# AnnSeidel/genometools

Measured on AMD Instinct MI355X. Metric: Gbp/s ESA build (suf+lcp+bwt), 3 Gbp DNA, 1/2/4/8 MI355X; bit-exact vs CPU, higher is better.
Workload: dtype u64; 1 GPU; human-like DNA (2% N, 24 seqs, repeats) n=3000000000 seed=43 -suf -lcp -bwt (BASELINE.json configs[2]); parallelism=1 device, pair_suffixes=341032298, tied_suffixes=390540711, refine_rounds=9, maxbranchdepth=8256

## Files before the change

### genometools_amd/csrc/esa_engine.hip

```cpp
#include <stdarg.h>
#include <stdlib.h>
#include <chrono>
#include <type_traits>
#include <utility>
#include <vector>
#include "../../include/gtamd_esa.h"
#include "esa_prims.h"
#include "esa_devutil.h"
#include "esa_own.h"

static thread_local char g_err[1024] = "";
void gtamd_set_error(const char *fmt, ...) {
  va_list ap;
  va_start(ap, fmt);
  vsnprintf(g_err, sizeof g_err, fmt, ap);
  va_end(ap);
}
extern "C" const char *gtamd_esa_last_error(void) { return g_err; }

extern "C" int gtamd_device_count(void) {
  GTAMD_ABI_BEGIN
  int n = 0;
  if (hipGetDeviceCount(&n) != hipSuccess) return 0;
  return n;
  GTAMD_ABI_END(0)
}

extern "C" int gtamd_abi_selftest(uint64_t host_bytes) {
  GTAMD_ABI_BEGIN
  std::vector<u8> probe((size_t) host_bytes);
  if (!probe.empty()) probe[probe.size() - 1] = 1;
  return probe.empty() ? 0 : (int) probe[probe.size() - 1] - 1;
  GTAMD_ABI_END(-1)
}

// ... 2449 lines not shown
  if (const char *e = getenv("GTAMD_APPLY_EARLY")) sw.apply_early = atoi(e);
  if (sw.apply_early < 0 || sw.apply_early > 2) sw.apply_early = 0;
  if (const char *e = getenv("GTAMD_APPLY_WGS")) {
    const long v = atol(e);
    if (v >= 64 && v <= (1 << 22)) sw.apply_wgs = (u64) v;
    sw.apply_wgs_given = true;
  }
  if (const char *e = getenv("GTAMD_RANK_WINDOW_BITS")) {
    const int v = atoi(e);
    if (v >= 2 && v <= RW_BITS) sw.rank_window_bits = v;
  }
  sw.rank_all_windows = flag("GTAMD_RANK_ALL_WINDOWS", '1');
  sw.win_filter_global = flag("GTAMD_WIN_FILTER_LDS", '0');
  if (const char *e = getenv("GTAMD_PAIR_CHUNK")) {
    const int v = atoi(e);
    if (v >= 4 && v <= 1024) sw.pair_chunk = v;
  }
  if (const char *e = getenv("GTAMD_ROUND_STRIDE")) {
    const int v = atoi(e);
    if (v >= RT_STRIDE_MIN && v <= RT_TILE) sw.round_stride = (u32) v;
  }
  sw.debug = getenv("GTAMD_DEBUG") != nullptr;
  return sw;
}

struct gtamd_esa_ctx {
  int device = 0;
  u32 sigma = 0;
  int bits = 0;
  u64 max_n = 0, n = 0, N = 0;
  int readmode = 0;
  Stream st, st2;
  Event ev_sorted, ev_emitted, ev_applied;
  DevBuf tb_own, sp_own;
  Text text = {};
  bool have_text = false;
  DevBuf k0, k1, v0, v1;
  DevBuf isa_tmp;
  DevBuf rws;
  DevBuf msd;
  DevBuf suf, lcp, bwt;
  DevBuf tiebits, tiebits2;
  DevBuf arena;
  DevBuf arena_p;
  DevBuf xrecv;
  DevBuf winbuf;
  DevBuf lcpfull_buf;
  DevBuf partws;
  DevBuf posw;
  Dev<u64> llv;
  u64 llv_pairs = 0;
  Dev<u32> bck;
  u64 bck_codes = 0, bck_special = 0, bck_dist = 0;
  Dev<Stats> d_stats;
  Pinned<Stats> h_stats;
  Pinned<u32> h_counts;
  Pinned<u32> h_hist;
  u32 user_prefixlength = 0;
  u32 part = 0, numparts = 1;
  gtamd_allgather_fn comm_allgather = nullptr;
  gtamd_alltoallv_fn comm_alltoallv = nullptr;
  void (*comm_abort)(void *) = nullptr;
  void *comm_abort_user = nullptr;
  void *comm_user = nullptr;
  u64 NL = 0, index_offset = 0;
  Dev<u32> d_parthist;
// ... 37 lines not shown
                    "context holds %llu bytes already, %llu of the device's %llu "
                    "are free",
                    (unsigned long long) bytes, what,
                    (unsigned long long) c->alloc_bytes, (unsigned long long) mfree,
                    (unsigned long long) mtotal);
    return -1;
  }
  c->alloc_bytes += bytes;
  return 0;
}

extern "C" void gtamd_esa_destroy(gtamd_esa_ctx *c) {
  if (c == nullptr) return;
  (void) hipSetDevice(c->device);
  if (c->st != nullptr) (void) hipStreamSynchronize(c->st);
  if (c->st2 != nullptr) (void) hipStreamSynchronize(c->st2);
  delete c;
}

static u64 max_positions(int bits) {
  const int spare = bits == 2 ? Key<2>::SPARE_BITS : Key<5>::SPARE_BITS;
  const int total = 32 + spare > 40 ? 40 : 32 + spare;
  return 1ull << total;
}
constexpr u64 SINGLE_LIMIT = (1ull << 32) - 4096;

static int create_resources(gtamd_esa_ctx *c) {
  HIP_TRY(hipSetDevice(c->device));
  HIP_TRY(create(c->st, hipStreamNonBlocking));
  HIP_TRY(create(c->st2, hipStreamNonBlocking));
  HIP_TRY(create(c->ev_sorted, hipEventDisableTiming));
  HIP_TRY(create(c->ev_emitted, hipEventDisableTiming));
  HIP_TRY(create(c->ev_applied, hipEventDisableTiming));
  HIP_TRY(c->d_stats.alloc(sizeof(Stats)));
  HIP_TRY(c->h_stats.alloc(sizeof(Stats)));
  HIP_TRY(c->h_counts.alloc(4 * DEST_MAXPARTS * 4));
  HIP_TRY(c->h_hist.alloc(PART_BINS * 4));
  HIP_TRY(c->d_parthist.alloc(PART_BINS * 4));
  HIP_TRY(c->d_owner.alloc(PART_BINS));
  HIP_TRY(c->d_counts.alloc(4 * DEST_MAXPARTS * 4));
  for (Event &e : c->ev) HIP_TRY(create(e));
  for (Event &e : c->ev_scatter) HIP_TRY(create(e));
  return 0;
}

extern "C" gtamd_esa_ctx *gtamd_esa_create(int device, uint64_t max_n,
                                           uint32_t numofchars) {
  GTAMD_ABI_BEGIN
  if (gtamd_device_count() <= device || device < 0) {
    gtamd_set_error("no HIP device %d available (this library has no CPU "
                    "fallback)", device);
    return nullptr;
  }
  if (numofchars < 2 || numofchars > 28) {
    gtamd_set_error("alphabet size %u not supported (2..28)", numofchars);
    return nullptr;
  }
  const int bits = numofchars <= 4 ? 2 : 5;
  if (max_n + 1 >= max_positions(bits) - 4096) {
    gtamd_set_error("sequence of %llu symbols exceeds the position range of "
                    "this engine (%llu)", (unsigned long long) max_n,
                    (unsigned long long) max_positions(bits));
    return nullptr;
  }
  gtamd_esa_ctx *c = new gtamd_esa_ctx();
  c->device = device;
// ... 292 lines not shown
         scan_workspace_words(div_up(cap, 64)) + 64;
}
static int ensure_workspace(gtamd_esa_ctx *c, u64 cap, u32 want, bool dist) {
  const u64 pad = cap + 8;
  TRY(ensure_buf(c, c->k0, pad * 8, "sort keys"));
  TRY(ensure_buf(c, c->k1, pad * 8, "sort keys"));
  TRY(ensure_buf(c, c->v0, pad * 4, "sort values"));
  TRY(ensure_buf(c, c->v1, pad * 4, "sort values"));
  TRY(ensure_buf(c, c->rws, rws_words_for(cap) * 4, "the radix workspace"));
  TRY(ensure_buf(c, c->tiebits, (div_up(cap, 64) + 2) * 8, "the tie bitmap"));
  if (want & GTAMD_WANT_SUF) TRY(ensure_buf(c, c->suf, pad * 8, "the suffix table"));
  if (want & GTAMD_WANT_LCP) TRY(ensure_buf(c, c->lcp, pad, "the lcp table"));
  if (want & GTAMD_WANT_BWT) TRY(ensure_buf(c, c->bwt, pad, "the bwt table"));
  if (dist) TRY(ensure_buf(c, c->isa_tmp, pad * 8, "the exchange scratch"));
  return 0;
}

static int msd_cbits_max(u64 N) {
  const int c = bits_for(N > 1 ? N - 1 : 1) - 24;
  return c < 0 ? 0 : (c > 8 ? 8 : c);
}
static int msd_choose_cbits(u64 N, int cmax, const float *penalty) {
  int best = cmax;
  float best_cost = 0.0f;
  for (int k = 1; k >= 0; k--) {
    const int c = cmax - 2 + k;
    if (c < 6) continue;
    const float gain = k == 1 ? 0.17f : 0.57f;
    const float cost = (penalty[k] - penalty[2]) / (float) N - gain;
    if (cost < best_cost) { best = c; best_cost = cost; }
  }
  return best;
}
struct MsdWs {
  u32 *hist, *scanws, *tcnt, *tfirst, *dtcnt, *dtfirst, *startA, *startB, *F, *scan2, *counters,
      *biglist, *giantlist, *crowdlist, *bndA;
  MsTile *desc;
  MdTile *dtiles;
  u64 *firstkey, *lastkey;
  u32 rows, tilesB_ub, tilesC_ub, tilesD_ub;
  u64 nf;
};
static u64 msd_carve(u64 N, int cb, u8 *base, MsdWs *w) {
  const u32 ntA = (u32) div_up(N, MS_TILE);
  w->tilesB_ub = ntA + 256;
  w->tilesC_ub = ntA + MSD_PARENTS;
  w->tilesD_ub = (u32) (2 * div_up(N, MS_TILE)) + MSD_PARENTS + 8;
  w->rows = w->tilesC_ub + 2;
  w->nf = (u64) MSD_PARENTS << cb;
  Bump b;
  b.base = base;
  b.off = 0;
  w->hist = b.take<u32>((u64) w->rows * 256);
  w->scanws = b.take<u32>(radix_rows_workspace_words(w->rows));
  w->desc = b.take<MsTile>(w->tilesC_ub);
  w->tcnt = b.take<u32>(MSD_PARENTS + 8);
  w->tfirst = b.take<u32>(MSD_PARENTS + 8);
  w->dtcnt = b.take<u32>(MSD_PARENTS + 8);
  w->dtfirst = b.take<u32>(MSD_PARENTS + 8);
  w->startA = b.take<u32>(256 + 8);
  w->bndA = b.take<u32>(256 * MSD_BLOCKS);
  w->startB = b.take<u32>(MSD_PARENTS + 8);
  w->F = b.take<u32>(w->nf + 8);
  w->scan2 = b.take<u32>(scan_workspace_words(w->nf + 1) + 64);
  w->counters = b.take<u32>(16);
  w->dtiles = b.take<MdTile>(w->tilesD_ub);
  w->firstkey = b.take<u64>(w->tilesD_ub);
  w->lastkey = b.take<u64>(w->tilesD_ub);
  w->biglist = b.take<u32>(w->tilesD_ub);
  w->crowdlist = b.take<u32>(w->tilesD_ub);
  w->giantlist = b.take<u32>((u64) (N / MS_TILE) + 8);
  return b.off + 256;
}

static int msd_level_prepare(gtamd_esa_ctx *c, const MsdWs &w, const u32 *pstart, u32 np, int cb,
                             u32 tiles_ub, const u32 *kin, const u64 *ein, u32 *cstart) {
  hipStream_t st = c->st;
  k_msd_tilecount<<<(np + 1 + 255) / 256, 256, 0, st>>>(pstart, 0, np, (u32) MS_TILE, w.tcnt);
  HIP_TRY(hipGetLastError());
  TRY(scan_u32(SCAN_SUM, w.tcnt, w.tfirst, (u64) np + 1, false, w.scan2, st));
  k_msd_tiledesc<<<(tiles_ub + 255) / 256, 256, 0, st>>>(pstart, w.tfirst, np, tiles_ub, w.desc);
  HIP_TRY(hipGetLastError());
  if (ein != nullptr)
    k_msd_hist_lvl<u64><<<tiles_ub + 1, MS_THREADS, 0, st>>>(ein, w.desc, tiles_ub, 32 - cb, w.hist);
  else
    k_msd_hist_lvl<u32><<<tiles_ub + 1, MS_THREADS, 0, st>>>(kin, w.desc, tiles_ub, 32 - cb, w.hist);
  HIP_TRY(hipGetLastError());
  TRY(radix_scan_tile_rows(w.hist, tiles_ub + 1, w.scanws, st));
  const u64 nchild = (u64) np << cb;
  k_msd_tot<<<(u32) div_up(nchild + 1, 256), 256, 0, st>>>(w.hist, w.tfirst, np, cb, cstart);
  HIP_TRY(hipGetLastError());
  TRY(scan_u32(SCAN_SUM, cstart, cstart, nchild + 1, false, w.scan2, st));
  return 0;
}

struct MsdPartSrc {
  const u64 *ck;
  const u32 *cp32;
  u64 index_offset;
  const unsigned long long *prev_key;
  int has_prev;
};
template <int FMT>
static int msd_sort_emit(gtamd_esa_ctx *c, const Switches &sw, u32 want, u32 prefixlength, u64 N,
// ... 102 lines not shown
      HIP_TRY(hipMemcpy(dt.data(), w.dtiles, (size_t) ntD * sizeof(MdTile), hipMemcpyDeviceToHost));
    u32 largest = 0;
    for (const MdTile &d : dt) largest = d.end - d.begin > largest ? d.end - d.begin : largest;
    fprintf(stderr, "gtamd: %smsd level D: packed=%d pack_cap=%u tiles=%u largest=%u\n", dpre,
            (int) packed, pack_cap, ntD, largest);
  }
  std::vector<MdTile> giants(ngiant);
  std::vector<u32> giant_t(ngiant);
  if (ngiant > 0) {
    HIP_TRY(hipMemcpy(giant_t.data(), w.giantlist, (size_t) ngiant * 4, hipMemcpyDeviceToHost));
    for (u32 i = 0; i < ngiant; i++)
      HIP_TRY(hipMemcpy(&giants[i], w.dtiles + giant_t[i], sizeof(MdTile), hipMemcpyDeviceToHost));
  }
  if (cb > 0) {
    k_msd_scatter_lvl<2, false><<<((w.tilesC_ub + 7u) >> 3) * 8u, MS_THREADS, 0, st>>>(
        kb, nullptr, pb, nullptr, nullptr, 0, w.desc, w.tilesC_ub, w.hist, w.tfirst, w.F, cb,
        32 - cb, ka, pa);
    HIP_TRY(hipGetLastError());
  }
  MsdOut o;
  o.suf = (want & GTAMD_WANT_SUF) ? c->suf.as<u64>() : nullptr;
  o.lcp = (want & GTAMD_WANT_LCP) ? c->lcp.as<u8>() : nullptr;
  o.bwt = (want & GTAMD_WANT_BWT) ? c->bwt.as<u8>() : nullptr;
  o.sa = pf;
  o.tiebits = c->tiebits.as<u64>();
  o.firstkey = w.firstkey;
  o.lastkey = w.lastkey;
  o.stats = c->d_stats;
  o.prefixlength = prefixlength;
  o.index_offset = src != nullptr ? src->index_offset : 0;
  o.val_is_index = src != nullptr && src->cp32 == nullptr;
  if (o.val_is_index) o.suf = nullptr;
  HIP_TRY(hipMemsetAsync(o.tiebits, 0, (div_up(N, 64) + 2) * 8, st));
  if (ntD > 0) {
    HIP_TRY(hipEventRecord(c->ev_scatter[0], st));
    const int force_radix = sw.msd_radix ? 1 : 0;
    k_msd_local<FMT><<<stride_grid(ntD), MS_THREADS, 0, st>>>(kf, pf, w.dtiles, ntD, cb,
                                                        force_radix, sw.msd_bin_limit,
                                                        w.crowdlist, w.counters, o);
    HIP_TRY(hipEventRecord(c->ev_scatter[1], st));
    HIP_TRY(hipGetLastError());
    k_msd_local_radix<FMT><<<ntD < 2048u ? ntD : 2048u, MS_THREADS, 0, st>>>(kf, pf, w.dtiles,
                                                                        w.crowdlist, w.counters,
                                                                        cb, o);
    HIP_TRY(hipGetLastError());
    if (sw.debug) {
      HIP_TRY(hipMemcpyAsync(hc + 6, w.counters + 4, 4, hipMemcpyDeviceToHost, st));
      HIP_TRY(hipStreamSynchronize(st));
      fprintf(stderr, "gtamd: %smsd local: radix_runs=%u force_radix=%d bin_limit=%u\n", dpre, hc[6],
              force_radix, sw.msd_bin_limit);
    }
  }
  if (nbig > 0) {
    k_msd_big<FMT><<<nbig < 2048u ? nbig : 2048u, MS_THREADS, 0, st>>>(kf, pf, ko, po, w.dtiles,
                                                                w.biglist, w.counters, cb, o);
    HIP_TRY(hipGetLastError());
  }
  for (u32 i = 0; i < ngiant; i++) {
    const MdTile g = giants[i];
    const u64 cnt = g.end - g.begin;
    const int shifts[4] = {FMT == 1 ? 8 : 3, FMT == 1 ? 14 : 11, FMT == 1 ? 20 : 19, FMT == 1 ? 26 : 27};
    const int widths[4] = {FMT == 1 ? 6 : 8, FMT == 1 ? 6 : 8, FMT == 1 ? 6 : 8, FMT == 1 ? 6 : 5};
    int nev = 0;
    TRY(radix_sort_pairs<u32, u32>(kf + g.begin, pf + g.begin, ko + g.begin, po + g.begin, cnt,
                                   shifts, widths, 4, c->rws.as<u32>(), st, nullptr, &nev));
    k_msd_emit_run<FMT><<<(u32) div_up(cnt, MS_TILE), MS_THREADS, 0, st>>>(kf, pf, giant_t[i], g.begin,
                                                                     (u32) cnt, g.s16, o);
    HIP_TRY(hipGetLastError());
  }
  if (ntD > 0) {
    k_msd_seams<FMT><<<(ntD + 255) / 256, 256, 0, st>>>(w.dtiles, ntD, src != nullptr ? src->prev_key : nullptr,
                                                   src != nullptr ? src->has_prev : 0, o);
    HIP_TRY(hipGetLastError());
  }
  *sa_out = pf;
  *fkey = reinterpret_cast<u64 *>(ko);
  *fval = po;
  *local_entries = N - nbigentries;
  c->stats.msd_big_entries = nbigentries;
  return 0;
}

static int passes_for(int from, int to, int *ps, int *pw) {
  int cnt = 0;
  for (int b = from; b < to; b += 8) {
    ps[cnt] = b;
    pw[cnt] = to - b < 8 ? to - b : 8;
    cnt++;
  }
  return cnt;
}

template <typename T>
static std::vector<u32> range_cuts(const T *bins, u32 R) {
  u64 nsamp = 0;
  for (int b = 0; b < PART_BINS; b++) nsamp += bins[b];
  std::vector<u32> cut(R + 1);
  cut[0] = 0;
// ... 1639 lines not shown
```

### genometools_amd/csrc/esa_msd.h

```cpp
#pragma once
#include "esa_msd_blocks.h"

constexpr int MS_TILE = 4096;
constexpr int MS_THREADS = 512;
constexpr int MS_WAVES = MS_THREADS / 64;
constexpr int MS_ITEMS = MS_TILE / MS_THREADS;
constexpr int MS_WCHUNK = MS_ITEMS * 64;
constexpr int MS_PAD = 520;
constexpr u32 MSD_PARENTS = 65536;
constexpr u32 MSD_STRIDE = 3328;
constexpr int MD_ITEMS = 8;
constexpr u32 MD_CAP = MD_ITEMS * MS_THREADS;
constexpr u32 MSD_BIG_MAX = 1u << 19;

struct MsTile {
  u32 start;
  u32 segvalid;
};
struct MdTile {
  u32 begin, end;
  u32 s16;
  u32 pad;
};
struct MsdOut {
// ... 990 lines not shown
        atomicAdd(&counters[2], n);
        atomicMax(&counters[1], n);
      }
      tiles[idx] = d;
    }
    t++;
  };
  for (u32 j0 = 0; j0 < nr; j0 += 8) {
    u32 nx[8];
#pragma unroll
    for (int k = 0; k < 8; k++) nx[k] = j0 + k < nr ? F[lo + j0 + k + 1] : 0u;
#pragma unroll
    for (int k = 0; k < 8; k++) {
      const u32 j = j0 + (u32) k;
      if (j < nr) {
        const u32 next = nx[k];
        if (prev > begin && next - begin > cap) {
          close(prev, j);
          begin = prev;
          jstart = j;
        }
        prev = next;
      }
    }
  }
  if (prev > begin) close(prev, nr);
  if (!EMIT) cnt[s] = t;
}

__device__ __forceinline__ u32 k2_letters(u32 k2) {
  const u32 dc = (k2 >> 3) & 31u;
  return dc == 0 ? 20u : (dc == 31u ? 0u : 20u - dc);
}
template <int FMT, bool INTERIOR>
__device__ __forceinline__ u32 msd_emit_quad(const u32 *s_key, const u32 *s_val, int i0, u32 cnt,
                                             u64 g0, u32 base, bool has_prev, u32 prevk2, u32 s16,
                                             const MsdOut &o, MsdAcc &acc) {
  u32 k[4], pv[4];
#pragma unroll
  for (int c = 0; c < 4; c++) {
    const int i = i0 + c;
    const bool ok = INTERIOR || (i >= 0 && i < (int) cnt);
    k[c] = ok ? s_key[i] + base : 0u;
    pv[c] = ok ? s_val[i] : 0u;
  }
  const u32 prevk = (INTERIOR || i0 > 0) ? s_key[i0 - 1] + base : prevk2;
  u32 lcpv[4] = {0, 0, 0, 0}, tiemask = 0;
  const u64 chi = (u64) s16 << 24;
  u32 da = FMT == 1 ? ((prevk & 32u) ? p5_letters(chi | (prevk >> 8)) : 9u) : k2_letters(prevk);
#pragma unroll
  for (int c = 0; c < 4; c++) {
    const int i = i0 + c;
    const bool ok = INTERIOR || (i >= 0 && i < (int) cnt);
    const bool have_a = INTERIOR || i > 0 || has_prev;
    const u32 a = (c == 0 || (!INTERIOR && i == 0)) ? prevk : k[c - 1], b = k[c];
    if (!INTERIOR && c > 0 && i == 0)
      da = FMT == 1 ? ((prevk & 32u) ? p5_letters(chi | (prevk >> 8)) : 9u) : k2_letters(prevk);
    const u32 db = FMT == 1 ? ((b & 32u) ? p5_letters(chi | (b >> 8)) : 9u) : k2_letters(b);
    const u32 x = (a ^ b) >> 8;
    u32 m;
    bool tie;
    if (FMT == 1) {
      m = p5_common(chi | (a >> 8), chi | (b >> 8));
      tie = x == 0 && db == 9u;
    } else {
      m = x ? 8u + ((u32) __clz((int) x) - 8u) / 2u : 20u;
      tie = x == 0 && ((a | b) & 0xF8u) == 0;
    }
    u32 l = m < da ? m : da;
    l = l < db ? l : db;
    if (!have_a) { l = 0; tie = false; }
    da = db;
    if (!ok) continue;
    lcpv[c] = l;
    if (tie) {
      tiemask |= 1u << c;
      acc.ties++;
    } else {
      if (have_a) {
        acc.mx = l > acc.mx ? l : acc.mx;
        if (db >= o.prefixlength) acc.sum += l;
      }
      if (pv[c] == 0 && !o.val_is_index) o.stats->longest = o.index_offset + g0 + (u64) c;
    }
  }
  if (INTERIOR || (i0 >= 0 && i0 + 4 <= (int) cnt)) {
    if (o.suf != nullptr) {
      *reinterpret_cast<ulonglong2 *>(o.suf + g0) = make_ulonglong2(pv[0], pv[1]);
      *reinterpret_cast<ulonglong2 *>(o.suf + g0 + 2) = make_ulonglong2(pv[2], pv[3]);
    }
    *reinterpret_cast<uint4 *>(o.sa + g0) = make_uint4(pv[0], pv[1], pv[2], pv[3]);
    if (o.lcp != nullptr)
      *reinterpret_cast<u32 *>(o.lcp + g0) =
          lcpv[0] | (lcpv[1] << 8) | (lcpv[2] << 16) | (lcpv[3] << 24);
    if (o.bwt != nullptr) {
      u32 bw = 0;
#pragma unroll
      for (int c = 0; c < 4; c++)
        bw |= (u32) (FMT == 1 ? Pay<5>::to_bwt(k[c] & 31u) : Pay<2>::to_bwt(k[c] & 7u)) << (8 * c);
      *reinterpret_cast<u32 *>(o.bwt + g0) = bw;
    }
  } else {
#pragma unroll
    for (int c = 0; c < 4; c++) {
      const int i = i0 + c;
      if (i < 0 || i >= (int) cnt) continue;
      if (o.suf != nullptr) o.suf[g0 + c] = pv[c];
      o.sa[g0 + c] = pv[c];
      if (o.lcp != nullptr) o.lcp[g0 + c] = (u8) lcpv[c];
      if (o.bwt != nullptr) o.bwt[g0 + c] = FMT == 1 ? Pay<5>::to_bwt(k[c] & 31u) : Pay<2>::to_bwt(k[c] & 7u);
    }
  }
  return tiemask;
}

template <int FMT>
__device__ __forceinline__ void msd_emit(const u32 *s_key, const u32 *s_val, u32 cnt, u64 gbeg,
                                         u32 base, bool has_prev, u32 prevk2, u32 s16,
                                         const MsdOut &o, u32 *s_bits, MsdAcc &acc) {
  static_assert(Key<2>::SYMS == 20 && Key<2>::DMAX == 31, "the layout msd_full spells out");
  const int tid = threadIdx.x;
  const u32 off64 = (u32) (gbeg & 63);
  const u32 nbw = (cnt + off64 + 63u) >> 6;
  for (u32 i = tid; i < 2u * nbw; i += MS_THREADS) s_bits[i] = 0;
  lds_barrier();
  const u32 mis = (u32) (gbeg & 3);
  const u32 nquads = (cnt + mis + 3u) >> 2;
  const u64 gq = gbeg - mis;
  for (u32 q = tid; q < nquads; q += MS_THREADS) {
    const int i0 = (int) (4u * q) - (int) mis;
    const u64 g0 = gq + 4ull * q;
    u32 tiemask;
    if (i0 >= 1 && i0 + 4 <= (int) cnt)
      tiemask = msd_emit_quad<FMT, true>(s_key, s_val, i0, cnt, g0, base, has_prev, prevk2, s16, o, acc);
// ... 27 lines not shown
    acc.ties += __shfl_xor(acc.ties, d, 64);
    const u32 ot = __shfl_xor(acc.mx, d, 64);
    acc.mx = ot > acc.mx ? ot : acc.mx;
  }
  if (lane == 0) { s_sum[w] = acc.sum; s_ties[w] = acc.ties; s_max[w] = acc.mx; }
  __syncthreads();
  if (threadIdx.x == 0) {
    unsigned long long S = 0, T = 0;
    u32 M = 0;
    for (int i = 0; i < (int) (blockDim.x >> 6); i++) {
      S += s_sum[i]; T += s_ties[i]; M = s_max[i] > M ? s_max[i] : M;
    }
    if (S) atomicAdd(&stats->lcpsum, S);
    if (T) atomicAdd(&stats->numties, T);
    if (M) atomicMax(&stats->maxlcp, M);
  }
}

__device__ __forceinline__ void msd_run_bits(const u32 *__restrict__ kin, u32 begin, u32 end,
                                             int cb, u32 &base, int &nbits) {
  if (cb == 0) { base = 0; nbits = 32; return; }
  const int csh = 32 - cb;
  const u32 f0 = kin[begin] >> csh, f1 = kin[end - 1] >> csh;
  base = f0 << csh;
  nbits = csh + (f1 > f0 ? 32 - __clz((int) (f1 - f0)) : 0);
}

constexpr int MD_BITS = 9;
constexpr int MD_RADIX = 1 << MD_BITS;
static_assert(MD_RADIX == MS_THREADS, "one thread per digit in the scan");

constexpr int MD_BINBITS = 12;
constexpr int MD_BINS = 1 << MD_BINBITS;
constexpr u32 MD_BIN_LIMIT_DEFAULT = 128;

__device__ __forceinline__ u32 md_base(const u32 *s_binw, u32 bin) {
  return (s_binw[bin >> 1] >> ((bin & 1u) * 16u)) & 0xFFFFu;
}

template <int FMT>
__global__ __launch_bounds__(MS_THREADS, 4) void k_msd_local(
    const u32 *__restrict__ kin, const u32 *__restrict__ pin, const MdTile *__restrict__ tiles,
    u32 ntiles, int cb, int force_radix, u32 bin_limit, u32 *__restrict__ crowdlist,
    u32 *__restrict__ counters, MsdOut o) {
  __shared__ u32 s_key[MS_TILE];
  __shared__ u32 s_val[MS_TILE];
  __shared__ __attribute__((aligned(16))) u32 s_binw[MD_BINS / 2 + 8];
  __shared__ u32 s_scan[MS_WAVES];
  __shared__ u32 s_bits[(MS_TILE + 128) / 32];
  static_assert(MD_BINS / 2 == 4 * MS_THREADS, "four counter words per thread in the scan");
  const int tid = threadIdx.x, lane = tid & 63, w = tid >> 6;
  u32 *s_c = s_key;
  MsdAcc acc;
  acc.sum = acc.ties = 0;
  acc.mx = 0;
  u32 key[MD_ITEMS], val[MD_ITEMS], rk[MD_ITEMS];
  const MdTile none = {0u, 0u, 0u, 0u};
  MdTile td = none;
  u32 t = blockIdx.x;
  if (t < ntiles) td = tiles[t];
  auto fetch = [&](const MdTile &x) {
    const u32 cnt = x.end - x.begin;
    if (cnt == 0 || cnt > MD_CAP) return;
    const u32 items = (cnt + MS_THREADS - 1) / MS_THREADS, wchunk = items * 64u;
    const u32 *kp = kin + x.begin;
    const u32 *pp = pin + x.begin;
#pragma unroll
    for (int j = 0; j < MD_ITEMS; j++) {
      const u32 e = (u32) w * wchunk + (u32) j * 64 + lane;
      if ((u32) j < items && e < cnt) {
        key[j] = kp[e];
        val[j] = pp[e];
      }
    }
  };
  fetch(td);
  while (t < ntiles) {
    const u32 tn = t + gridDim.x;
    MdTile tdn = none;
    if (tn < ntiles) tdn = tiles[tn];
    const u32 cnt = td.end - td.begin;
    bool skip = cnt == 0 || cnt > MD_CAP;
    u32 base = 0;
    if (!skip) {
      const int csh = 32 - cb;
      const u32 span = td.pad >> 16;
      base = cb ? (td.pad & 0xFFFFu) << csh : 0u;
      const int nbits = cb ? csh + (span > 1u ? 32 - __clz((int) (span - 1u)) : 0) : 32;
      const u32 items = (cnt + MS_THREADS - 1) / MS_THREADS, wchunk = items * 64u;
      const u32 e0 = (u32) w * wchunk + lane;
      constexpr int PB = MsdFmt<FMT>::PB;
      const int sb = nbits - PB;
      const int binshift = sb > MD_BINBITS ? nbits - MD_BINBITS : PB;
      const u32 lowmask = sb > MD_BINBITS ? (1u << (binshift - PB)) - 1u : 0u;
      for (int i = tid; i < MD_BINS / 8 + 2; i += MS_THREADS)
        reinterpret_cast<uint4 *>(s_binw)[i] = make_uint4(0, 0, 0, 0);
      lds_barrier();
#pragma unroll
      for (int j = 0; j < MD_ITEMS; j++) {
        if ((u32) j < items && e0 + 64u * j < cnt) {
          key[j] -= base;
          const u32 bin = key[j] >> binshift;
          const u32 old = atomicAdd(&s_binw[bin >> 1], (bin & 1u) ? 65536u : 1u);
          rk[j] = (bin & 1u) ? old >> 16 : old & 0xFFFFu;
        }
      }
      lds_barrier();
      {
        const uint4 q0 = reinterpret_cast<uint4 *>(s_binw)[tid];
        u32 wd[4] = {q0.x, q0.y, q0.z, q0.w};
        u32 run = 0, mx = 0;
#pragma unroll
        for (int k = 0; k < 4; k++) {
          const u32 c0 = wd[k] & 0xFFFFu, c1 = wd[k] >> 16;
          mx = c0 > mx ? c0 : mx;
          mx = c1 > mx ? c1 : mx;
          wd[k] = run | ((run + c0) << 16);
          run += c0 + c1;
        }
        const u32 pre = ms_scan_excl(run, s_scan) * 0x10001u;
        reinterpret_cast<uint4 *>(s_binw)[tid] =
            make_uint4(wd[0] + pre, wd[1] + pre, wd[2] + pre, wd[3] + pre);
        if (tid == 0) s_binw[MD_BINS / 2] = cnt;
        if (mx > bin_limit || force_radix) s_binw[MD_BINS / 2 + 1] = 1u;
      }
      lds_barrier();
      if (s_binw[MD_BINS / 2 + 1] != 0) {
        if (tid == 0) {
          crowdlist[atomicAdd(&counters[4], 1u)] = t;
          atomicAdd(&o.stats->crowded, (unsigned long long) cnt);
        }
        skip = true;
      } else {
        u32 b0[MD_ITEMS];
#pragma unroll
        for (int j = 0; j < MD_ITEMS; j++)
          b0[j] = ((u32) j < items && e0 + 64u * j < cnt) ? md_base(s_binw, key[j] >> binshift) : 0u;
#pragma unroll
        for (int j = 0; j < MD_ITEMS; j++)
          if ((u32) j < items && e0 + 64u * j < cnt)
            s_c[b0[j] + rk[j]] = (((key[j] >> PB) & lowmask) << 12) | (e0 + 64u * j);
        lds_barrier();
        u32 b1[MD_ITEMS], m0[MD_ITEMS], m1[MD_ITEMS];
#pragma unroll
        for (int j = 0; j < MD_ITEMS; j++) {
          const bool ok = (u32) j < items && e0 + 64u * j < cnt;
          b1[j] = ok ? md_base(s_binw, (key[j] >> binshift) + 1u) : 1u;
          m0[j] = s_c[b0[j]];
        }
#pragma unroll
        for (int j = 0; j < MD_ITEMS; j++) m1[j] = s_c[b0[j] + 1u < b1[j] ? b0[j] + 1u : b0[j]];
#pragma unroll
        for (int j = 0; j < MD_ITEMS; j++) {
          const u32 c = (((key[j] >> PB) & lowmask) << 12) | (e0 + 64u * j);
          u32 r = b0[j] + (m0[j] < c ? 1u : 0u) + (m1[j] < c ? 1u : 0u);
          if (b0[j] + 1u >= b1[j]) r = b0[j];
          if (b1[j] - b0[j] > 2u)
            for (u32 q = b0[j] + 2u; q < b1[j]; q++) r += s_c[q] < c ? 1u : 0u;
          rk[j] = r;
        }
        lds_barrier();
#pragma unroll
        for (int j = 0; j < MD_ITEMS; j++) {
          if ((u32) j < items && e0 + 64u * j < cnt) {
            s_key[rk[j]] = key[j];
            s_val[rk[j]] = val[j];
          }
        }
        lds_barrier();
      }
    }
    fetch(tdn);
    if (!skip) {
      if (tid == 0) {
        o.firstkey[t] = msd_full<FMT>(td.s16, s_key[0] + base);
        o.lastkey[t] = msd_full<FMT>(td.s16, s_key[cnt - 1] + base);
      }
      msd_emit<FMT>(s_key, s_val, cnt, td.begin, base, false, 0u, td.s16, o, s_bits, acc);
    }
    t = tn;
    td = tdn;
  }
  __syncthreads();
  msd_acc_flush(acc, o.stats);
}

template <int FMT>
__global__ __launch_bounds__(MS_THREADS) void k_msd_local_radix(
    const u32 *__restrict__ kin, const u32 *__restrict__ pin, const MdTile *__restrict__ tiles,
    const u32 *__restrict__ crowdlist, const u32 *__restrict__ counters, int cb, MsdOut o) {
  __shared__ u32 s_key[MS_TILE];
  __shared__ u32 s_val[MS_TILE];
  __shared__ u16 s_cnt_mem[MS_WAVES * MD_RADIX];
  __shared__ u32 s_scan[MS_WAVES];
  __shared__ u32 s_bits[(MS_TILE + 128) / 32];
  const int tid = threadIdx.x, lane = tid & 63, w = tid >> 6;
  ms_vu16 *s_cnt = (ms_vu16 *) s_cnt_mem;
  ms_vu16 *cnt_w = s_cnt + w * MD_RADIX;
  const u32 ncrowd = counters[4];
  MsdAcc acc;
  acc.sum = acc.ties = 0;
  acc.mx = 0;
  for (u32 ci = blockIdx.x; ci < ncrowd; ci += gridDim.x) {
    const u32 t = crowdlist[ci];
    const MdTile td = tiles[t];
// ... 192 lines not shown
            dk[g] = k + base;
            dp[g] = s_val[e];
          }
        }
        __syncthreads();
      }
      u32 *x = sk; sk = dk; dk = x;
      x = sp; sp = dp; dp = x;
    }
    u32 prevkey = 0;
    for (u32 c0 = 0; c0 < cnt; c0 += (u32) MS_TILE) {
      const u32 valid = cnt - c0 < (u32) MS_TILE ? cnt - c0 : (u32) MS_TILE;
#pragma unroll
      for (int j = 0; j < MS_ITEMS; j++) {
        const u32 e = (u32) j * MS_THREADS + tid;
        if (e < valid) {
          s_key[e] = sk[c0 + e] - base;
          s_val[e] = sp[c0 + e];
        }
      }
      __syncthreads();
      if (tid == 0) {
        if (c0 == 0) o.firstkey[t] = msd_full<FMT>(td.s16, s_key[0] + base);
        if (c0 + valid == cnt) o.lastkey[t] = msd_full<FMT>(td.s16, s_key[valid - 1] + base);
      }
      const u32 lastk = s_key[valid - 1] + base;
      msd_emit<FMT>(s_key, s_val, valid, (u64) td.begin + c0, base, c0 > 0, prevkey, td.s16, o, s_bits, acc);
      prevkey = lastk;
    }
  }
  msd_acc_flush(acc, o.stats);
}

template <int FMT>
__global__ __launch_bounds__(MS_THREADS) void k_msd_emit_run(
    const u32 *__restrict__ kin, const u32 *__restrict__ pin, u32 t, u32 begin, u32 cnt, u32 s16,
    MsdOut o) {
  __shared__ u32 s_key[MS_TILE];
  __shared__ u32 s_val[MS_TILE];
  __shared__ u32 s_bits[(MS_TILE + 128) / 32];
  const int tid = threadIdx.x;
  MsdAcc acc;
  acc.sum = acc.ties = 0;
  acc.mx = 0;
  const u32 c0 = blockIdx.x * (u32) MS_TILE;
  const u32 valid = cnt - c0 < (u32) MS_TILE ? cnt - c0 : (u32) MS_TILE;
#pragma unroll
  for (int j = 0; j < MS_ITEMS; j++) {
    const u32 e = (u32) j * MS_THREADS + tid;
    if (e < valid) {
      s_key[e] = kin[(u64) begin + c0 + e];
      s_val[e] = pin[(u64) begin + c0 + e];
    }
  }
  __syncthreads();
  if (tid == 0) {
    if (c0 == 0) o.firstkey[t] = msd_full<FMT>(s16, s_key[0]);
    if (c0 + valid == cnt) o.lastkey[t] = msd_full<FMT>(s16, s_key[valid - 1]);
  }
  const u32 prevkey = c0 > 0 ? kin[(u64) begin + c0 - 1] : 0u;
  msd_emit<FMT>(s_key, s_val, valid, (u64) begin + c0, 0u, c0 > 0, prevkey, s16, o, s_bits, acc);
  msd_acc_flush(acc, o.stats);
}

template <int FMT>
__global__ __launch_bounds__(256) void k_msd_seams(const MdTile *__restrict__ tiles, u32 ntiles,
// ... 36 lines not shown
```

Measured before the change: 26.75 Gbp/s.

## Skip constant digits in giant radix sorts, prefetch next tile, nontemporal stores

Before the giant-bucket radix sorts run, a small kernel ORs together the XOR of each giant's keys against its first key. The host then drops any radix pass whose digit is constant across the bucket, and copies the result back when an odd number of passes remains. Separately, the MSD local kernel now fetches the next tile's keys before processing the current one to overlap load latency. Emit stores switch to nontemporal vector stores, and statistics are accumulated per quad before updating. The risks are added host synchronisation on an event and extra register pressure from the prefetch buffers.

```diff
diff --git a/genometools_amd/csrc/esa_engine.hip b/genometools_amd/csrc/esa_engine.hip
--- a/genometools_amd/csrc/esa_engine.hip
+++ b/genometools_amd/csrc/esa_engine.hip
@@ -1,6 +1,8 @@
 #include <stdarg.h>
 #include <stdlib.h>
+#include <array>
 #include <chrono>
+#include <string>
 #include <type_traits>
 #include <utility>
 #include <vector>
@@ -2516,6 +2518,7 @@
   int readmode = 0;
   Stream st, st2;
   Event ev_sorted, ev_emitted, ev_applied;
+  Event ev_look;
   DevBuf tb_own, sp_own;
   Text text = {};
   bool have_text = false;
@@ -2619,6 +2622,7 @@
   HIP_TRY(create(c->ev_sorted, hipEventDisableTiming));
   HIP_TRY(create(c->ev_emitted, hipEventDisableTiming));
   HIP_TRY(create(c->ev_applied, hipEventDisableTiming));
+  HIP_TRY(create(c->ev_look, hipEventDisableTiming));
   HIP_TRY(c->d_stats.alloc(sizeof(Stats)));
   HIP_TRY(c->h_stats.alloc(sizeof(Stats)));
   HIP_TRY(c->h_counts.alloc(4 * DEST_MAXPARTS * 4));
@@ -2977,9 +2981,12 @@
   }
   return best;
 }
+constexpr u32 MSD_GIANT_LOOK = 256;
+constexpr u32 MSD_GIANT_HC = 16;
+static_assert(MSD_GIANT_HC + MSD_GIANT_LOOK <= 4 * DEST_MAXPARTS, "h_counts holds them");
 struct MsdWs {
   u32 *hist, *scanws, *tcnt, *tfirst, *dtcnt, *dtfirst, *startA, *startB, *F, *scan2, *counters,
-      *biglist, *giantlist, *crowdlist, *bndA;
+      *biglist, *giantlist, *giantbits, *crowdlist, *bndA;
   MsTile *desc;
   MdTile *dtiles;
   u64 *firstkey, *lastkey;
@@ -3015,6 +3022,7 @@
   w->biglist = b.take<u32>(w->tilesD_ub);
   w->crowdlist = b.take<u32>(w->tilesD_ub);
   w->giantlist = b.take<u32>((u64) (N / MS_TILE) + 8);
+  w->giantbits = b.take<u32>(MSD_GIANT_LOOK);
   return b.off + 256;
 }
 
@@ -3183,6 +3191,22 @@
   o.val_is_index = src != nullptr && src->cp32 == nullptr;
   if (o.val_is_index) o.suf = nullptr;
   HIP_TRY(hipMemsetAsync(o.tiebits, 0, (div_up(N, 64) + 2) * 8, st));
+  const int gshifts[4] = {FMT == 1 ? 8 : 3, FMT == 1 ? 14 : 11, FMT == 1 ? 20 : 19, FMT == 1 ? 26 : 27};
+  const int gwidths[4] = {FMT == 1 ? 6 : 8, FMT == 1 ? 6 : 8, FMT == 1 ? 6 : 8, FMT == 1 ? 6 : 5};
+  const u32 nlook = ngiant < MSD_GIANT_LOOK ? ngiant : MSD_GIANT_LOOK;
+  if (nlook > 0) {
+    HIP_TRY(hipMemsetAsync(w.giantbits, 0, (size_t) nlook * 4, st));
+    for (u32 i = 0; i < nlook; i++) {
+      const u32 cnt = giants[i].end - giants[i].begin;
+      const u32 nb = (cnt + 4095u) / 4096u;
+      k_msd_diffbits<<<nb < 2048u ? nb : 2048u, 256, 0, st>>>(kf + giants[i].begin, cnt, w.giantbits + i);
+      HIP_TRY(hipGetLastError());
+    }
+    HIP_TRY(hipMemcpyAsync(hc + MSD_GIANT_HC, w.giantbits, (size_t) nlook * 4, hipMemcpyDeviceToHost, st));
+    HIP_TRY(hipEventRecord(c->ev_look, st));
+  }
+  std::vector<std::array<int, 4>> giant_sh(ngiant), giant_wd(ngiant);
+  std::vector<int> giant_np(ngiant);
   if (ntD > 0) {
     HIP_TRY(hipEventRecord(c->ev_scatter[0], st));
     const int force_radix = sw.msd_radix ? 1 : 0;
@@ -3195,11 +3219,25 @@
                                                                         w.crowdlist, w.counters,
                                                                         cb, o);
     HIP_TRY(hipGetLastError());
+    if (nlook > 0) HIP_TRY(hipEventSynchronize(c->ev_look));
+    std::string gp = ngiant > 0 ? "" : "none";
+    for (u32 i = 0; i < ngiant; i++) {
+      const u32 differ = i < nlook ? hc[MSD_GIANT_HC + i] : ~0u;
+      int np = 0;
+      for (int p = 0; p < 4; p++) {
+        if (((differ >> gshifts[p]) & ((1u << gwidths[p]) - 1u)) == 0) continue;
+        giant_sh[i][np] = gshifts[p];
+        giant_wd[i][np] = gwidths[p];
+        np++;
+      }
+      giant_np[i] = np;
+      gp += (i > 0 ? "," : "") + std::to_string(np);
+    }
     if (sw.debug) {
       HIP_TRY(hipMemcpyAsync(hc + 6, w.counters + 4, 4, hipMemcpyDeviceToHost, st));
       HIP_TRY(hipStreamSynchronize(st));
-      fprintf(stderr, "gtamd: %smsd local: radix_runs=%u force_radix=%d bin_limit=%u\n", dpre, hc[6],
-              force_radix, sw.msd_bin_limit);
+      fprintf(stderr, "gtamd: %smsd local: radix_runs=%u force_radix=%d bin_limit=%u giant_passes=%s\n",
+              dpre, hc[6], force_radix, sw.msd_bin_limit, gp.c_str());
     }
   }
   if (nbig > 0) {
@@ -3210,11 +3248,16 @@
   for (u32 i = 0; i < ngiant; i++) {
     const MdTile g = giants[i];
     const u64 cnt = g.end - g.begin;
-    const int shifts[4] = {FMT == 1 ? 8 : 3, FMT == 1 ? 14 : 11, FMT == 1 ? 20 : 19, FMT == 1 ? 26 : 27};
-    const int widths[4] = {FMT == 1 ? 6 : 8, FMT == 1 ? 6 : 8, FMT == 1 ? 6 : 8, FMT == 1 ? 6 : 5};
-    int nev = 0;
-    TRY(radix_sort_pairs<u32, u32>(kf + g.begin, pf + g.begin, ko + g.begin, po + g.begin, cnt,
-                                   shifts, widths, 4, c->rws.as<u32>(), st, nullptr, &nev));
+    if (giant_np[i] > 0) {
+      int nev = 0;
+      TRY(radix_sort_pairs<u32, u32>(kf + g.begin, pf + g.begin, ko + g.begin, po + g.begin, cnt,
+                                     giant_sh[i].data(), giant_wd[i].data(), giant_np[i],
+                                     c->rws.as<u32>(), st, nullptr, &nev));
+      if (giant_np[i] & 1) {
+        HIP_TRY(hipMemcpyAsync(kf + g.begin, ko + g.begin, cnt * 4, hipMemcpyDeviceToDevice, st));
+        HIP_TRY(hipMemcpyAsync(pf + g.begin, po + g.begin, cnt * 4, hipMemcpyDeviceToDevice, st));
+      }
+    }
     k_msd_emit_run<FMT><<<(u32) div_up(cnt, MS_TILE), MS_THREADS, 0, st>>>(kf, pf, giant_t[i], g.begin,
                                                                      (u32) cnt, g.s16, o);
     HIP_TRY(hipGetLastError());
diff --git a/genometools_amd/csrc/esa_msd.h b/genometools_amd/csrc/esa_msd.h
--- a/genometools_amd/csrc/esa_msd.h
+++ b/genometools_amd/csrc/esa_msd.h
@@ -1046,6 +1046,34 @@
   const u32 dc = (k2 >> 3) & 31u;
   return dc == 0 ? 20u : (dc == 31u ? 0u : 20u - dc);
 }
+__device__ __forceinline__ void msd_acc_quad(u32 tiemask, u32 qsum, u32 qmx, u32 zeromask, u64 g0,
+                                             const MsdOut &o, MsdAcc &acc) {
+  acc.ties += (u32) __popc(tiemask);
+  acc.sum += qsum;
+  acc.mx = qmx > acc.mx ? qmx : acc.mx;
+  if (zeromask != 0 && !o.val_is_index)
+    o.stats->longest = o.index_offset + g0 + (u64) (__ffs((int) zeromask) - 1);
+}
+template <int FMT>
+__device__ __forceinline__ void msd_store_quad(const u32 (&k)[4], const u32 (&pv)[4],
+                                               const u32 (&lcpv)[4], u64 g0, const MsdOut &o) {
+  typedef u32 v4u __attribute__((ext_vector_type(4)));
+  if (o.suf != nullptr) {
+    __builtin_nontemporal_store((v4u){pv[0], 0u, pv[1], 0u}, reinterpret_cast<v4u *>(o.suf + g0));
+    __builtin_nontemporal_store((v4u){pv[2], 0u, pv[3], 0u}, reinterpret_cast<v4u *>(o.suf + g0 + 2));
+  }
+  __builtin_nontemporal_store((v4u){pv[0], pv[1], pv[2], pv[3]}, reinterpret_cast<v4u *>(o.sa + g0));
+  if (o.lcp != nullptr)
+    __builtin_nontemporal_store(lcpv[0] | (lcpv[1] << 8) | (lcpv[2] << 16) | (lcpv[3] << 24),
+                                reinterpret_cast<u32 *>(o.lcp + g0));
+  if (o.bwt != nullptr) {
+    u32 bw = 0;
+#pragma unroll
+    for (int c = 0; c < 4; c++)
+      bw |= (u32) (FMT == 1 ? Pay<5>::to_bwt(k[c] & 31u) : Pay<2>::to_bwt(k[c] & 7u)) << (8 * c);
+    __builtin_nontemporal_store(bw, reinterpret_cast<u32 *>(o.bwt + g0));
+  }
+}
 template <int FMT, bool INTERIOR>
 __device__ __forceinline__ u32 msd_emit_quad(const u32 *s_key, const u32 *s_val, int i0, u32 cnt,
                                              u64 g0, u32 base, bool has_prev, u32 prevk2, u32 s16,
@@ -1059,7 +1087,7 @@
     pv[c] = ok ? s_val[i] : 0u;
   }
   const u32 prevk = (INTERIOR || i0 > 0) ? s_key[i0 - 1] + base : prevk2;
-  u32 lcpv[4] = {0, 0, 0, 0}, tiemask = 0;
+  u32 lcpv[4] = {0, 0, 0, 0}, tiemask = 0, qsum = 0, qmx = 0, zeromask = 0;
   const u64 chi = (u64) s16 << 24;
   u32 da = FMT == 1 ? ((prevk & 32u) ? p5_letters(chi | (prevk >> 8)) : 9u) : k2_letters(prevk);
 #pragma unroll
@@ -1089,31 +1117,17 @@
     lcpv[c] = l;
     if (tie) {
       tiemask |= 1u << c;
-      acc.ties++;
     } else {
       if (have_a) {
-        acc.mx = l > acc.mx ? l : acc.mx;
-        if (db >= o.prefixlength) acc.sum += l;
-      }
-      if (pv[c] == 0 && !o.val_is_index) o.stats->longest = o.index_offset + g0 + (u64) c;
-    }
-  }
+        qmx = l > qmx ? l : qmx;
+        if (db >= o.prefixlength) qsum += l;
+      }
+      if (pv[c] == 0) zeromask |= 1u << c;
+    }
+  }
+  msd_acc_quad(tiemask, qsum, qmx, zeromask, g0, o, acc);
   if (INTERIOR || (i0 >= 0 && i0 + 4 <= (int) cnt)) {
-    if (o.suf != nullptr) {
-      *reinterpret_cast<ulonglong2 *>(o.suf + g0) = make_ulonglong2(pv[0], pv[1]);
-      *reinterpret_cast<ulonglong2 *>(o.suf + g0 + 2) = make_ulonglong2(pv[2], pv[3]);
-    }
-    *reinterpret_cast<uint4 *>(o.sa + g0) = make_uint4(pv[0], pv[1], pv[2], pv[3]);
-    if (o.lcp != nullptr)
-      *reinterpret_cast<u32 *>(o.lcp + g0) =
-          lcpv[0] | (lcpv[1] << 8) | (lcpv[2] << 16) | (lcpv[3] << 24);
-    if (o.bwt != nullptr) {
-      u32 bw = 0;
-#pragma unroll
-      for (int c = 0; c < 4; c++)
-        bw |= (u32) (FMT == 1 ? Pay<5>::to_bwt(k[c] & 31u) : Pay<2>::to_bwt(k[c] & 7u)) << (8 * c);
-      *reinterpret_cast<u32 *>(o.bwt + g0) = bw;
-    }
+    msd_store_quad<FMT>(k, pv, lcpv, g0, o);
   } else {
 #pragma unroll
     for (int c = 0; c < 4; c++) {
@@ -1207,7 +1221,9 @@
 
 constexpr int MD_BINBITS = 12;
 constexpr int MD_BINS = 1 << MD_BINBITS;
+constexpr int MD_SCANW = MD_BINS / 2 / MS_THREADS;
 constexpr u32 MD_BIN_LIMIT_DEFAULT = 128;
+constexpr int MD_MATES = 2;
 
 __device__ __forceinline__ u32 md_base(const u32 *s_binw, u32 bin) {
   return (s_binw[bin >> 1] >> ((bin & 1u) * 16u)) & 0xFFFFu;
@@ -1223,7 +1239,8 @@
   __shared__ __attribute__((aligned(16))) u32 s_binw[MD_BINS / 2 + 8];
   __shared__ u32 s_scan[MS_WAVES];
   __shared__ u32 s_bits[(MS_TILE + 128) / 32];
-  static_assert(MD_BINS / 2 == 4 * MS_THREADS, "four counter words per thread in the scan");
+  static_assert(MD_BINS / 2 == MD_SCANW * MS_THREADS && MD_SCANW % 4 == 0,
+                "whole uint4s of counter words per thread in the scan");
   const int tid = threadIdx.x, lane = tid & 63, w = tid >> 6;
   u32 *s_c = s_key;
   MsdAcc acc;
@@ -1234,7 +1251,7 @@
   MdTile td = none;
   u32 t = blockIdx.x;
   if (t < ntiles) td = tiles[t];
-  auto fetch = [&](const MdTile &x) {
+  auto fetch = [&](const MdTile &x, u32 (&fk)[MD_ITEMS], u32 (&fv)[MD_ITEMS]) {
     const u32 cnt = x.end - x.begin;
     if (cnt == 0 || cnt > MD_CAP) return;
     const u32 items = (cnt + MS_THREADS - 1) / MS_THREADS, wchunk = items * 64u;
@@ -1244,12 +1261,20 @@
     for (int j = 0; j < MD_ITEMS; j++) {
       const u32 e = (u32) w * wchunk + (u32) j * 64 + lane;
       if ((u32) j < items && e < cnt) {
-        key[j] = kp[e];
-        val[j] = pp[e];
+        fk[j] = kp[e];
+        fv[j] = pp[e];
       }
     }
   };
-  fetch(td);
+  {
+    u32 fk[MD_ITEMS], fv[MD_ITEMS];
+    fetch(td, fk, fv);
+#pragma unroll
+    for (int j = 0; j < MD_ITEMS; j++) {
+      asm volatile("v_mov_b32 %0, %1" : "=v"(key[j]) : "v"(fk[j]));
+      asm volatile("v_mov_b32 %0, %1" : "=v"(val[j]) : "v"(fv[j]));
+    }
+  }
   while (t < ntiles) {
     const u32 tn = t + gridDim.x;
     MdTile tdn = none;
@@ -1257,6 +1282,8 @@
     const u32 cnt = td.end - td.begin;
     bool skip = cnt == 0 || cnt > MD_CAP;
     u32 base = 0;
+    u32 nk[MD_ITEMS], nv[MD_ITEMS];
+    fetch(tdn, nk, nv);
     if (!skip) {
       const int csh = 32 - cb;
       const u32 span = td.pad >> 16;
@@ -1282,11 +1309,15 @@
       }
       lds_barrier();
       {
-        const uint4 q0 = reinterpret_cast<uint4 *>(s_binw)[tid];
-        u32 wd[4] = {q0.x, q0.y, q0.z, q0.w};
+        u32 wd[MD_SCANW];
+#pragma unroll
+        for (int k = 0; k < MD_SCANW; k += 4) {
+          const uint4 q0 = reinterpret_cast<uint4 *>(s_binw)[tid * (MD_SCANW / 4) + k / 4];
+          wd[k] = q0.x; wd[k + 1] = q0.y; wd[k + 2] = q0.z; wd[k + 3] = q0.w;
+        }
         u32 run = 0, mx = 0;
 #pragma unroll
-        for (int k = 0; k < 4; k++) {
+        for (int k = 0; k < MD_SCANW; k++) {
           const u32 c0 = wd[k] & 0xFFFFu, c1 = wd[k] >> 16;
           mx = c0 > mx ? c0 : mx;
           mx = c1 > mx ? c1 : mx;
@@ -1294,8 +1325,10 @@
           run += c0 + c1;
         }
         const u32 pre = ms_scan_excl(run, s_scan) * 0x10001u;
-        reinterpret_cast<uint4 *>(s_binw)[tid] =
-            make_uint4(wd[0] + pre, wd[1] + pre, wd[2] + pre, wd[3] + pre);
+#pragma unroll
+        for (int k = 0; k < MD_SCANW; k += 4)
+          reinterpret_cast<uint4 *>(s_binw)[tid * (MD_SCANW / 4) + k / 4] =
+              make_uint4(wd[k] + pre, wd[k + 1] + pre, wd[k + 2] + pre, wd[k + 3] + pre);
         if (tid == 0) s_binw[MD_BINS / 2] = cnt;
         if (mx > bin_limit || force_radix) s_binw[MD_BINS / 2 + 1] = 1u;
       }
@@ -1316,22 +1349,27 @@
           if ((u32) j < items && e0 + 64u * j < cnt)
             s_c[b0[j] + rk[j]] = (((key[j] >> PB) & lowmask) << 12) | (e0 + 64u * j);
         lds_barrier();
-        u32 b1[MD_ITEMS], m0[MD_ITEMS], m1[MD_ITEMS];
+        u32 b1[MD_ITEMS], m[MD_MATES][MD_ITEMS];
 #pragma unroll
         for (int j = 0; j < MD_ITEMS; j++) {
           const bool ok = (u32) j < items && e0 + 64u * j < cnt;
           b1[j] = ok ? md_base(s_binw, (key[j] >> binshift) + 1u) : 1u;
-          m0[j] = s_c[b0[j]];
-        }
-#pragma unroll
-        for (int j = 0; j < MD_ITEMS; j++) m1[j] = s_c[b0[j] + 1u < b1[j] ? b0[j] + 1u : b0[j]];
+          m[0][j] = s_c[b0[j]];
+        }
+#pragma unroll
+        for (int s = 1; s < MD_MATES; s++)
+#pragma unroll
+          for (int j = 0; j < MD_ITEMS; j++)
+            m[s][j] = s_c[b0[j] + (u32) s < b1[j] ? b0[j] + (u32) s : b1[j] - 1u];
 #pragma unroll
         for (int j = 0; j < MD_ITEMS; j++) {
           const u32 c = (((key[j] >> PB) & lowmask) << 12) | (e0 + 64u * j);
-          u32 r = b0[j] + (m0[j] < c ? 1u : 0u) + (m1[j] < c ? 1u : 0u);
-          if (b0[j] + 1u >= b1[j]) r = b0[j];
-          if (b1[j] - b0[j] > 2u)
-            for (u32 q = b0[j] + 2u; q < b1[j]; q++) r += s_c[q] < c ? 1u : 0u;
+          u32 r = b0[j];
+#pragma unroll
+          for (int s = 0; s < MD_MATES; s++)
+            r += (b0[j] + (u32) s < b1[j] && m[s][j] < c) ? 1u : 0u;
+          if (b1[j] - b0[j] > (u32) MD_MATES)
+            for (u32 q = b0[j] + (u32) MD_MATES; q < b1[j]; q++) r += s_c[q] < c ? 1u : 0u;
           rk[j] = r;
         }
         lds_barrier();
@@ -1345,7 +1383,11 @@
         lds_barrier();
       }
     }
-    fetch(tdn);
+#pragma unroll
+    for (int j = 0; j < MD_ITEMS; j++) {
+      asm volatile("v_mov_b32 %0, %1" : "=v"(key[j]) : "v"(nk[j]));
+      asm volatile("v_mov_b32 %0, %1" : "=v"(val[j]) : "v"(nv[j]));
+    }
     if (!skip) {
       if (tid == 0) {
         o.firstkey[t] = msd_full<FMT>(td.s16, s_key[0] + base);
@@ -1604,6 +1646,17 @@
   msd_acc_flush(acc, o.stats);
 }
 
+__global__ __launch_bounds__(256) void k_msd_diffbits(const u32 *__restrict__ k, u32 cnt,
+                                                      u32 *__restrict__ out) {
+  const u32 k0 = k[0];
+  u32 d = 0;
+  for (u64 i = (u64) blockIdx.x * 256u + threadIdx.x; i < cnt; i += (u64) gridDim.x * 256u)
+    d |= k[i] ^ k0;
+#pragma unroll
+  for (int s = 32; s >= 1; s >>= 1) d |= __shfl_xor(d, s, 64);
+  if ((threadIdx.x & 63) == 0 && d != 0) atomicOr(out, d);
+}
+
 template <int FMT>
 __global__ __launch_bounds__(MS_THREADS) void k_msd_emit_run(
     const u32 *__restrict__ kin, const u32 *__restrict__ pin, u32 t, u32 begin, u32 cnt, u32 s16,
```

Result: no change. 26.74 Gbp/s (-0.0%).
